# BaratiLab/LNS-Latent-Neural-PDE-Solver

Measured on AMD Instinct MI355X. Metric: rollout-steps/sec (encode+N latent steps+decode), NS2d 128^2 3-ch, higher is better.
Workload: dtype f32 (f16x2 split operands on the fp16 MFMA pipe, fp32 accumulate; fp32 tensors in HBM); 1 GPU; NS2d 128x128 3-channel, 64-step latent rollout, batch=64 per GPU (BASELINE.json configs[1]); preset=ns2d_128, batch_per_gpu=64, rollout_steps=64, global_batch=64, parallelism=trajectory-sharded x1, streams=propagator + 3 decode streams per GPU

## Files before the change

lns-latent-neural-pde-solver_amd/csrc/conv3_up2q.inc:

```
#define CONVUQ_SLAB 8192
#define CONVUQ_STEP 2
#define CONVUQ_EPS_BYTES 32768

size_t convuq_lds_bytes(const ConvArgs& a) {
    const size_t ns = a.Cin_pad / 8, pp1 = (size_t)a.PH * a.PW + 1;
    return ns * pp1 * 32 + CONVUQ_EPS_BYTES + ((size_t)a.Cin_pad * 2 + 64) * 4 + 16 + 64;
}
bool convuq_fits(const ConvArgs& a) {
    return a.ks == 3 && a.stride == 1 && a.dil == 1 && a.up2 && a.wb != nullptr && a.Cin_pad >= 16 && a.Cin_pad <= 64 &&
           (a.Cin_pad % 16) == 0 && (long)a.PH * a.PW <= 256 && !a.x_oct && a.b0 == 0 && a.res == nullptr &&
           (long)a.Cout * a.Hout * a.Wout * 4 < (1L << 31) && convuq_lds_bytes(a) <= 80 * 1024;
}

template <bool FUSE2>
__global__ __launch_bounds__(256, 2) void conv3_up2q_kernel(ConvArgs a) {
    constexpr int NTHR = 256, TM = 64, KC = 8, MT = 2, NT = 1, UB = 32, SLAB = CONVUQ_SLAB, NS_MAX = 8, STEP = CONVUQ_STEP;
    constexpr int NWQ = STEP * SLAB / 16 / NTHR;
    static_assert(2 * STEP * SLAB <= CONVUQ_EPS_BYTES && 18944 <= CONVUQ_EPS_BYTES, "the ring covers the epilogue scratch it aliases");
    extern __shared__ __attribute__((aligned(16))) char smem[];
    const int PH = a.PH, PW = a.PW, PLANE = PH * PW, PP1 = PLANE + 1;
    const int ns = a.Cin_pad / KC;
    const int xs_bytes = PP1 * UB;
    char* Xres = smem;
    char* ring = Xres + ns * xs_bytes;
    float* ssl = reinterpret_cast<float*>(ring + CONVUQ_EPS_BYTES);
    float* addv = ssl + a.Cin_pad * 2;
    unsigned* wmax = reinterpret_cast<unsigned*>(addv + 64);

    const int tid = threadIdx.x, lane = tid & 63, wn = tid >> 6;
    const int l31 = lane & 31, kh = lane >> 5;
    const int b = blockIdx.y;
    const int ct = blockIdx.x % a.cout_tiles, tile = blockIdx.x / a.cout_tiles;
    const int tx = tile % a.tiles_x, ty = tile / a.tiles_x;
    const int BW = 1 << a.bw_log2, BH = 128 >> a.bw_log2;
// ... 39 lines not shown
    };
    load_half(0);
    const int nstep = ns / STEP;
    u32x4 wq[NWQ];
    auto load_w = [&](int q) __attribute__((always_inline)) {
        const int qc = q < 4 * nstep ? q : 4 * nstep - 1;
        const int ph = qc / nstep, sp0 = (qc - ph * nstep) * STEP;
#pragma unroll
        for (int i = 0; i < NWQ; ++i) {
            const int idx = tid + i * NTHR, st = sp0 + (idx >> 9);
            wq[i] = __builtin_amdgcn_raw_buffer_load_b128(wr, (idx & 511) * 16, (st * 4 + ph) * SLAB, 0);
        }
    };
    auto write_w = [&](int slot) __attribute__((always_inline)) {
#pragma unroll
        for (int i = 0; i < NWQ; ++i) *reinterpret_cast<u32x4*>(ring + slot * (STEP * SLAB) + (tid + i * NTHR) * 16) = wq[i];
    };
    load_w(0);
    {
        float addreg = 0.0f;
        if (tid < TM) {
            const int co = ct * TM + tid, cc = co < a.Cout ? co : 0;
            addreg = (a.bias ? a.bias[cc] : 0.0f) + (a.badd ? a.badd[(long)b * a.Cout + cc] : 0.0f);
        }
        stage_ss_bound(a, b, ssl, wmax, tid, NTHR);
        if (tid < TM) addv[tid] = addreg;
    }
    __syncthreads();
    float xinv = 1.0f;
    uok *= f16x2_scale(block_bound(a, wmax), xinv);

    auto stage_half = [&](auto mode_tag, int h) __attribute__((always_inline)) {
        constexpr int MODE = decltype(mode_tag)::value;
#pragma unroll
        for (int sl = 0; sl < HS; ++sl) {
            const int s = h * HS + sl;
            if (s < ns) {
                unsigned hq[4], lq[4];
#pragma unroll
                for (int cp = 0; cp < 4; ++cp) {
                    float t[2];
#pragma unroll
                    for (int e = 0; e < 2; ++e) {
                        float v = pv[sl * KC + 2 * cp + e];
                        if (MODE >= 1) { const float2 st = *reinterpret_cast<const float2*>(ssl + 2 * (s * KC + 2 * cp + e)); v = v * st.x + st.y; }
                        if (MODE == 2) v = swish_fast(v);
// ... 2 lines not shown
                    split2_pair_f16(t[0], t[1], hq[cp], lq[cp]);
                }
                char* dst = Xres + s * xs_bytes + uslot;
                *reinterpret_cast<uint4*>(dst) = make_uint4(hq[0], hq[1], hq[2], hq[3]);
                *reinterpret_cast<uint4*>(dst + 16) = make_uint4(lq[0], lq[1], lq[2], lq[3]);
            }
        }
    };
    auto stage_all = [&](auto mode_tag) __attribute__((always_inline)) {
        stage_half(mode_tag, 0);
        if (ns > HS) { load_half(1); stage_half(mode_tag, 1); }
    };
    if (pro_mode == 2) stage_all(std::integral_constant<int, 2>{});
    else if (pro_mode == 1) stage_all(std::integral_constant<int, 1>{});
    else stage_all(std::integral_constant<int, 0>{});
    write_w(0);
    load_w(1);
    __syncthreads();

    const int p = wn * 32 + l31;
    const int boff = ((p >> a.bw_log2) * PW + (p & (BW - 1))) * UB;
    const int aoff0 = ((0 + kh) * TM + l31) * 16, aoff1 = ((2 + kh) * TM + l31) * 16;
    unsigned am = 0u;
#pragma unroll 1
    for (int ph = 0; ph < 4; ++ph) {
        const int pa = ph >> 1, pb = ph & 1;
        const int lt0 = ((0 + pa) * PW + kh + pb) * UB, lt1 = ((1 + pa) * PW + kh + pb) * UB;
        f32x16 acc_hi[MT][NT], acc_lo[MT][NT];
#pragma unroll
        for (int mt = 0; mt < MT; ++mt)
#pragma unroll
            for (int r = 0; r < 16; ++r) { acc_hi[mt][0][r] = 0.0f; acc_lo[mt][0][r] = 0.0f; }
#pragma unroll 1
        for (int t = 0; t < nstep; ++t) {
#pragma unroll
            for (int u = 0; u < STEP; ++u) {
                const char* Wslot = ring + (t & 1) * (STEP * SLAB) + u * SLAB;
                const char* Xs = Xres + (t * STEP + u) * xs_bytes + boff;
                uint4 af[2][2][MT], bf[2][2];
#pragma unroll
                for (int j = 0; j < 2; ++j)
#pragma unroll
                    for (int sp = 0; sp < 2; ++sp) {
#pragma unroll
                        for (int mt = 0; mt < MT; ++mt)
                            af[j][sp][mt] = *reinterpret_cast<const uint4*>(Wslot + (j ? aoff1 : aoff0) + sp * (4 * TM * 16) + mt * (32 * 16));
                        bf[j][sp] = *reinterpret_cast<const uint4*>(Xs + (j ? lt1 : lt0) + sp * 16);
                    }
#pragma unroll
                for (int j = 0; j < 2; ++j) {
#define LNS_UQ3(ACC, SA, SB)                                                                          \
    _Pragma("unroll") for (int mt = 0; mt < MT; ++mt)                                                 \
        ACC[mt][0] = __builtin_amdgcn_mfma_f32_32x32x16_f16(__builtin_bit_cast(f16x8, af[j][SA][mt]), \
                                                            __builtin_bit_cast(f16x8, bf[j][SB]), ACC[mt][0], 0, 0, 0);
                    LNS_UQ3(acc_hi, 0, 0)
                    LNS_UQ3(acc_lo, 0, 1)
                    LNS_UQ3(acc_lo, 1, 0)
#undef LNS_UQ3
                }
            }
            if (t + 1 < nstep) {
                write_w((t + 1) & 1);
                if (t + 2 < nstep) load_w(ph * nstep + t + 2);
            }
            __syncthreads();
        }
        int pix[NT];
        {
            const int oy = 2 * (ty * BH + (p >> a.bw_log2)) + pa, ox = 2 * (tx * BW + (p & (BW - 1))) + pb;
            pix[0] = (oy < a.Hout && ox < a.Wout) ? oy * a.Wout + ox : -1;
        }
        convb_epilogue<NT, FUSE2, MT, true, true, true, true>(a, acc_hi, acc_lo, pix, b, ct, kh, l31, tid, ring, xinv, am,
                                                        (a.bias || a.badd) ? addv : nullptr, (ty * a.tiles_x + tx) * 4 + ph, nullptr, 4);
        if (ph < 3) {
            load_w((ph + 1) * nstep);
            __syncthreads();
            write_w(0);
            load_w((ph + 1) * nstep + 1);
            __syncthreads();
        }
    }
    if (a.amax_out) amax_publish_block(a.amax_out, b, am, wmax);
}

hipError_t launch_conv_up2q(const ConvArgs& a, hipStream_t s) {
    if (!convuq_fits(a) || !has_act_bound(a)) return hipErrorInvalidValue;
    dim3 grid(a.tiles_x * a.tiles_y * a.cout_tiles, a.B);
    const size_t lds = convuq_lds_bytes(a);
    if (a.w2) hipLaunchKernelGGL((conv3_up2q_kernel<true>), grid, dim3(256), lds, s, a);
    else hipLaunchKernelGGL((conv3_up2q_kernel<false>), grid, dim3(256), lds, s, a);
    return hipGetLastError();
}
```

lns-latent-neural-pde-solver_amd/csrc/lns_engine.cpp:

```cpp
#include <algorithm>
#include <cmath>
#include <cstdarg>
#include <cstdio>
#include <cstdlib>
#include <cstring>
#include <memory>
#include <mutex>
#include <tuple>
#include <stdexcept>
#include <type_traits>

#include "lns_engine.h"
#include "lns_fold.h"

#define LNS_MAX_BATCH 65535

namespace lns {
void build_model(lns_engine* e);

static thread_local std::string g_create_error;

static std::string fmt(const char* f, ...) {
    char buf[1024];
    va_list ap;
// ... 45 lines not shown
    out.resize(len);
    for (int p = 0; p < len; ++p) {
        int u = p - pad_lo;
        int src = -1;
        if (p < virt + pad_lo + pad_hi) {
            if (u < 0 || u >= virt) {
                if (mode == LNS_PAD_CIRCULAR) { u %= virt; if (u < 0) u += virt; }
                else u = -1;
            }
            if (u >= 0) src = nearest_src(u, in, virt, scale);
        }
        out[p] = src;
    }
}

static void pack_conv_weight(float* dst, const float* src, int cout_off, int cout, int cin, int k, int Cin_pad,
                             int Cout_pad) {
    const int taps = k * k;
    for (int co = 0; co < cout; ++co)
        for (int ci = 0; ci < cin; ++ci)
            for (int t = 0; t < taps; ++t)
                dst[((size_t)t * Cin_pad + ci) * Cout_pad + cout_off + co] = src[((size_t)co * cin + ci) * taps + t];
}

struct ConvGeom { int variant, bw_log2, tiles_x, tiles_y, cout_tiles, PH, PW, Hout, Wout, kc_log2, sel_kc_log2; };

static bool conv_geometry(ConvGeom& g, int B, int Cout, int Hv, int Wv, int k, int stride, int dil, const int* pad,
                          int kc_log2_pack, int Cout_pad, int force_variant, bool need_wgm1 = false,
                          bool allow_bf16x3 = false, int Cin = 1 << 30, bool f16x2 = false, bool allow_thin = false,
                          int force_bw_log2 = -1 ) {
    g.Hout = (Hv + pad[0] + pad[1] - dil * (k - 1) - 1) / stride + 1;
    g.Wout = (Wv + pad[2] + pad[3] - dil * (k - 1) - 1) / stride + 1;
    if (g.Hout <= 0 || g.Wout <= 0) return false;
    std::vector<int> cands;
    if (force_variant >= 0) cands = {force_variant};
    else if (Cout <= 32) cands = {CV_S32};
    else if (Cout <= 64) cands = need_wgm1 ? std::vector<int>{CV_L64, CV_M64} : std::vector<int>{CV_L64, CV_M64, CV_S64};
    else if (getenv("LNS_CONV_USE_128")) cands = {CV_L128, CV_M128, CV_S64};
    else cands = {CV_L64, CV_M64, CV_S64};
    static const bool no_bf16x3 = getenv("LNS_CONV_FP32_MFMA") != nullptr;
    const bool use_b = allow_bf16x3 && !no_bf16x3 && k == 3 && stride == 1 && Cout > 32;
    if (force_variant < 0 && use_b) {
        cands.insert(cands.begin(), f16x2 ? (int)CV_F64 : (int)CV_B64);
    }
    static const bool no_b1 = getenv("LNS_CONV1_FP32_MFMA") != nullptr;
    if (force_variant < 0 && allow_bf16x3 && !no_bf16x3 && !no_b1 && k == 1 && stride == 1 && Cout > 32 && Cin >= 16)
// ... 237 lines not shown
        static const long min_hw = getenv("LNS_GN_FUSE_MIN_HW") ? atol(getenv("LNS_GN_FUSE_MIN_HW")) : (no_fold ? 1024 : 256);
        Op* prod = nullptr;
        for (size_t i = plan->ops.size(); i-- > 0;) {
            const int ty = plan->ops[i].type;
            if (ty == OP_TRACE || ty == OP_CONDBLK || ty == OP_CONDBASE || ty == OP_VECLIN) continue;
            prod = &plan->ops[i];
            break;
        }
        static const bool no_ragged = getenv("LNS_GN_NO_RAGGED") != nullptr;
        const bool ragged1 = !no_fold && !no_ragged && prod && prod->type == OP_CONV && !prod->conv.up2 &&
                             prod->conv.tiles_x * prod->conv.tiles_y == 1 && x.H * x.W < GN_TILE_PIXELS;
        static const bool no_ragged_tiles = getenv("LNS_GN_NO_RAGGED_TILES") != nullptr;
        const bool raggedN = !no_fold && !no_ragged && !no_ragged_tiles && prod && prod->type == OP_CONV && !prod->conv.up2 && !ragged1 &&
                             x.H * x.W > GN_TILE_PIXELS;
        const bool prod_ok = prod && prod->type == OP_CONV &&
                             (prod->variant == CV_F64 || prod->variant == CV_F32 || prod->variant == CV_B64 ||
                              (prod->variant == CV_B1 && !no_fold && prod->conv.ct_per_block == 0 && !prod->conv.w2 &&
                               ((x.H * x.W) % GN_TILE_PIXELS == 0 || ragged1 || raggedN)));
        if (stat_scratch && (!premul || ragged1 || raggedN) && prod_ok &&
            prod->conv.y == as_ptr<float>(x.ptr) && prod->conv.Cout == x.C && ((long)x.H * x.W >= min_hw || ragged1)) {
            const ConvArgs& c = prod->conv;
            const int BW = 1 << c.bw_log2, BH = GN_TILE_PIXELS / BW;
            const int um = c.up2 ? 2 : 1;
            const int tiles = c.tiles_x * c.tiles_y * (c.up2 ? 4 : 1);
            const bool exact = c.ks == 1 ? (c.tiles_x * GN_TILE_PIXELS == x.H * x.W && c.tiles_y == 1)
                                         : (c.tiles_x * BW * um == x.W && c.tiles_y * BH * um == x.H);
            if ((exact || ragged1 || raggedN) && (size_t)B * tiles * x.C * 8 <= stat_cap) {
                const int cg = x.C / groups;
                static const int fold_tiles = getenv("LNS_GN_FOLD_TILES") ? atoi(getenv("LNS_GN_FOLD_TILES")) : 2;
                const bool foldable = !no_fold && (exact || ragged1) && tiles <= fold_tiles && x.C <= 512 && (!premul || groups == 1) &&
                                      (groups == 1 || (cg <= 64 && (cg & (cg - 1)) == 0));
                const int li = (int)lazy_ops.size();
                lazy_done.push_back(0); lazy_folded.push_back(0);
                const uint64_t region = take_stat_region(name, li);
                prod->conv.stat_part = as_ptr<float>(region);
                op.gn_tile_part = as_ptr<const float>(region);
                op.gn_tiles = tiles;
                op.gn_count = ragged1 ? x.H * x.W : GN_TILE_PIXELS;
                if (ragged1) prod->conv.stat_count = x.H * x.W;
                if (!exact && !ragged1) {
                    op.gn_count = -1;
                    op.gn_geom = GnTileGeom{c.tiles_x, c.bw_log2, x.H, x.W, c.ks == 1 ? 1 : 0};
                    prod->conv.stat_count = -1;
                }
                if (prod->chunk_group > 0)
                    for (Op& o : plan->ops)
                        if (o.type == OP_CONV && o.chunk_group == prod->chunk_group) {
                            o.conv.stat_part = prod->conv.stat_part; o.conv.stat_count = prod->conv.stat_count;
                        }
                op.bytes = 2.0 * B * tiles * x.C * 8;
                lazy_ops.push_back(op);
                if (foldable) { x.gn_lazy = li; return; }
                lazy_done[li] = 1;
            }
        }
        plan->ops.push_back(op);
    }

    static bool can_fuse_1x1(const ConvPack& first, const ConvPack& second) {
        static const bool off = getenv("LNS_NO_FUSE_1X1") != nullptr;
        return !off && first.cout == 64 && second.k == 1 && second.cin == 64 && second.cout == 64;
// ... 1 lines not shown
    TRef emit_conv(const TRef& in, int pack_id, int k, int stride, int dil, const int* pad, int my, int mx,
                   int act_out, const TRef* res, uint64_t badd, const TRef* out_forced, const std::string& name,
                   int fuse_pack = -1, bool want_amax = true) {
        const ConvPack& pk = e->packs[pack_id];
        if (pk.cin != in.C) throw std::runtime_error(fmt("%s: input has %d channels, conv expects %d", name.c_str(), in.C, pk.cin));
        int Hv = in.vH ? in.vH : in.H, Wv = in.vW ? in.vW : in.W;
        static const bool fp32_only = getenv("LNS_CONV_FP32_MFMA") != nullptr;
        const bool up2 = k == 3 && stride == 1 && dil == 1 && in.vH == 2 * in.H && in.vW == 2 * in.W && pk.has_wu && pk.f16 &&
                         pad[0] == 1 && pad[1] == 1 && pad[2] == 1 && pad[3] == 1 && in.bounded() && pk.cout > 32 && !fp32_only;
        if (up2) { Hv = in.H; Wv = in.W; }
        ConvGeom g;
        const bool thin_ok = !res && !badd && act_out == ACT_NONE && fuse_pack < 0 && !in.vH &&
                             (in.act == ACT_NONE || (in.act == ACT_SWISH && in.ss != 0));
        if (!conv_geometry(g, B, pk.cout, Hv, Wv, k, stride, dil, pad, pk.kc_log2, pk.Cout_pad, -1, fuse_pack >= 0,
                           pk.has_wb && in.bounded(), pk.cin, pk.f16, thin_ok))
            throw std::runtime_error("no conv tiling for " + name);
        if (up2 && g.variant == CV_F32 &&
            !conv_geometry(g, B, pk.cout, Hv, Wv, k, stride, dil, pad, pk.kc_log2, pk.Cout_pad, CV_F64, fuse_pack >= 0,
                           pk.has_wb && in.bounded(), pk.cin, pk.f16, thin_ok))
            throw std::runtime_error("no conv tiling for " + name);
        if (up2 && g.variant != CV_F64) throw std::runtime_error("phase form needs the f16x2 64-cout tiles: " + name);
        bool quad = false;
        {
            static const bool no_quad = getenv("LNS_UP2_QUAD") == nullptr || getenv("LNS_UP2_RESIDENT") != nullptr;
            ConvGeom gq;
            if (up2 && !no_quad && !res && pk.Cin_pad <= 64 && pk.Cin_pad % 16 == 0 &&
                conv_geometry(gq, B, pk.cout, Hv, Wv, k, stride, dil, pad, pk.kc_log2, pk.Cout_pad, CV_F64, fuse_pack >= 0,
                              pk.has_wb && in.bounded(), pk.cin, pk.f16, thin_ok, 4)) {
                ConvArgs t;
                memset(&t, 0, sizeof t);
                t.ks = 3; t.stride = 1; t.dil = 1; t.up2 = 1; t.wb = &t; t.Cin_pad = pk.Cin_pad; t.PH = gq.PH; t.PW = gq.PW;
                t.Cout = pk.cout; t.Hout = 2 * in.H; t.Wout = 2 * in.W;
                if (convuq_fits(t)) { g = gq; quad = true; }
            }
        }
        if (in.act == ACT_GELU && ((g.variant != CV_F64 && g.variant != CV_F32) || up2 || fuse_pack >= 0))
            throw NoGeluPrologue("GELU prologue is only built into the f16x2 3x3 kernel: " + name);
        if (up2) { g.Hout = 2 * in.H; g.Wout = 2 * in.W; }
        const ConvVariantInfo vi = conv_variant_info(g.variant);
        const int BW = 1 << g.bw_log2, BH = vi.TN / BW;
        std::vector<int> rm, cm;
        if (k == 3) {
            build_axis_map(rm, (g.tiles_y - 1) * BH * stride + g.PH, in.H, Hv, up2 ? 0.0f : in.sch, pad[0], pad[1], my);
            build_axis_map(cm, (g.tiles_x - 1) * BW * stride + g.PW, in.W, Wv, up2 ? 0.0f : in.scw, pad[2], pad[3], mx);
        } else if (in.vH) throw std::runtime_error("1x1 conv of a resized tensor is not supported: " + name);
        TRef out;
        if (out_forced) out = *out_forced;
        else out = alloc_t(pk.cout, g.Hout, g.Wout);
        if (out.C != pk.cout || out.H != g.Hout || out.W != g.Wout)
            throw std::runtime_error(fmt("%s: output shape mismatch (%d,%d,%d) vs (%d,%d,%d)", name.c_str(), out.C, out.H,
                                         out.W, pk.cout, g.Hout, g.Wout));
// ... 50 lines not shown
        a.unscale = (cv_is_f16x2_3x3(g.variant) || g.variant == CV_B1) ? 1.0f / (up2 ? pk.wscale_up : pk.wscale) : 1.0f;
        if (in.ss != 0 && in.gn_bound > 0.0f) { a.amax_in_const = in.gn_bound; a.bound_final = 1; }
        else {
            a.amax_in = as_ptr<const unsigned>(in.amax); a.amax_in_const = in.amax_const;
            if (!in.amax && in.ss == 0) a.bound_final = 1;
        }
        out.amax = 0; out.amax_const = 0.0f; out.gn_bound = 0.0f;
        if ((want_amax && g.variant != CV_THIN) || out_forced) { out.amax = new_amax(name); a.amax_out = as_ptr<unsigned>(out.amax); }
        a.Cin_pad = pk.Cin_pad; a.Cout_pad = pk.Cout_pad; a.kc_log2 = g.sel_kc_log2;
        a.tiles_x = g.tiles_x; a.tiles_y = g.tiles_y; a.cout_tiles = g.cout_tiles; a.bw_log2 = g.bw_log2;
        a.PH = g.PH; a.PW = g.PW; a.B = B;
        a.ph_magic = g.PH > 1 ? (unsigned)((0x100000000ull + g.PH - 1) / g.PH) : 0u;
        if (up2) {
            static const bool res = getenv("LNS_UP2_RESIDENT") != nullptr;
            if (res) { a.up2 = 2; if (!convur_fits(a)) a.up2 = 1; }
            if (quad && convuq_fits(a)) a.up2 = 3;
        }
        op.flops = 2.0 * B * g.Hout * g.Wout * (double)pk.cout * pk.cin * k * k;
        op.bytes = 4.0 * B * ((double)in.C * in.H * in.W + (double)pk.cout * g.Hout * g.Wout * (res ? 2 : 1));
        {
            const double tiles = (double)B * g.tiles_x * g.tiles_y * g.cout_tiles * vi.TM * vi.TN;
            if (cv_is_f16x2_3x3(g.variant)) {
                op.mfma_flops = tiles * pk.Cin_pad * (up2 ? 4.0 * 4.0 : 10.0) * 3.0 * 2.0;
                op.form = up2 ? (fuse_pack >= 0 ? "f16x2 3x3 four-tap phase form + fused 1x1" : "f16x2 3x3 four-tap phase form")
                              : (fuse_pack >= 0 ? "f16x2 3x3 nine-tap + fused 1x1" : "f16x2 3x3 nine-tap");
                if (fuse_pack >= 0) op.mfma_flops += tiles * (up2 ? 4.0 : 1.0) * 64.0 * 3.0 * 2.0;
            } else if (g.variant == CV_B64 || g.variant == CV_B32) {
                op.mfma_flops = tiles * pk.Cin_pad * 10.0 * 6.0 * 2.0; op.form = "bf16x3 3x3 nine-tap";
            } else if (g.variant == CV_B1) {
                const int cp32 = (pk.Cin_pad + 31) / 32 * 32;
                op.mfma_flops = tiles * cp32 * (convb1_is_f16() ? 3.0 : 6.0) * 2.0;
                op.form = a.ct_per_block ? "f16x2 1x1 input-stationary" : (fuse_pack >= 0 ? "f16x2 1x1 + fused 1x1" : "f16x2 1x1 streaming");
                if (fuse_pack >= 0) op.mfma_flops += tiles * 64.0 * 3.0 * 2.0;
            } else if (g.variant == CV_THIN) {
                op.form = "thin 1x1 projection (VALU)";
            } else {
                op.mfma_flops = tiles * pk.Cin_pad * (double)(k * k) * 2.0 + (fuse_pack >= 0 ? tiles * 64.0 * 2.0 : 0.0);
                op.form = k == 3 ? "fp32 MFMA 3x3" : "fp32 MFMA 1x1";
            }
        }
        if (fuse_pack >= 0) {
            const ConvPack& p2 = e->packs[fuse_pack];
            if (!can_fuse_1x1(pk, p2)) throw std::runtime_error("cannot fuse 1x1 into " + name);
            a.w2 = as_ptr<const float>(wt(p2.w_off));
            a.bias2 = p2.has_bias ? as_ptr<const float>(wt(p2.b_off)) : nullptr;
            a.Cout2_pad = p2.Cout_pad;
            {
// ... 1304 lines not shown
        if (n == "fa_fused" && (value < 0 || value > 3)) return LNS_EINVAL;
        const bool changed = n == "fa_fused" ? e->opt_fa_fused != (int)value : e->opt_fa_fused_gpb != (int)value;
        if (changed) {
            DeviceGuard dg(e);
            for (auto* m : {&e->enc_plans, &e->dec_plans}) {
                for (auto& kv : *m) if (kv.second.d_consts) (void)hipFree(kv.second.d_consts);
                m->clear();
            }
        }
        if (n == "fa_fused") e->opt_fa_fused = (int)value;
        else e->opt_fa_fused_gpb = (int)value;
    }
    else if (n == "fold_linear") {
        if (value != 0 && value != 1) { e->err = "fold_linear: 0 (the pair as it stands) or 1 (one conv on the composed weights)"; return LNS_EINVAL; }
        if (e->opt_fold_linear != (int)value) {
            DeviceGuard dg(e);
            for (auto* m : {&e->enc_plans, &e->dec_plans}) {
                for (auto& kv : *m) if (kv.second.d_consts) (void)hipFree(kv.second.d_consts);
                m->clear();
            }
        }
        e->opt_fold_linear = (int)value;
    }
    else if (n == "fa_chunk_mb") {
        if (value < 0 || value > 4096) return LNS_EINVAL;
        if (e->opt_fa_chunk_mb != (int)value) {
            DeviceGuard dg(e);
            for (auto* m : {&e->enc_plans, &e->dec_plans}) {
                for (auto& kv : *m) if (kv.second.d_consts) (void)hipFree(kv.second.d_consts);
                m->clear();
            }
        }
        e->opt_fa_chunk_mb = (int)value;
    }
    else if (n == "prop_priority") {
        if (e->opt_prop_priority != (value != 0)) { DeviceGuard dg(e); release_overlap_objects(e); }
        e->opt_prop_priority = value != 0;
    } else { e->err = "unknown option: " + n; return LNS_EINVAL; }
    e->ran.clear(); e->ran_ws = nullptr; e->ran_B = 0;
    return LNS_OK;
}

int lns_latent_shape(const lns_engine* e, int* C, int* H, int* W) {
    if (!e || e->enc.empty()) return LNS_EINVAL;
    if (C) *C = e->lat_C;
    if (H) *H = e->lat_H;
// ... 485 lines not shown
    if (name && cap > 0) { strncpy(name, t.name.c_str(), cap - 1); name[cap - 1] = 0; }
    if (ms) *ms = t.ms;
    if (launches) *launches = t.launches;
    if (flops) *flops = t.flops;
    if (bytes) *bytes = t.bytes;
    return LNS_OK;
}

int lns_timing_mfma_flops(const lns_engine* e, int i, double* mfma_flops) {
    if (e && i == -1 && mfma_flops) { *mfma_flops = e->timing_overhead_ms * 1e3; return LNS_OK; }
    if (!e || i < 0 || i >= (int)e->timing.size() || !mfma_flops) return LNS_EINVAL;
    *mfma_flops = e->timing[i].mfma_flops;
    return LNS_OK;
}

int lns_build_has(const char* feature) {
    if (!feature) return -1;
    if (!strcmp(feature, "experimental")) return build_has_experimental() ? 1 : 0;
    if (!strcmp(feature, "train_wgrad_split")) return 1;
    if (!strcmp(feature, "train_clip")) return 1;
    if (!strcmp(feature, "train_ops")) return 1;
    if (!strcmp(feature, "rollout_select")) return 1;
    if (!strcmp(feature, "rollout_ensemble")) return 1;
#ifdef LNS_DIAG
    if (!strcmp(feature, "diag")) return 1;
#else
    if (!strcmp(feature, "diag")) return 0;
#endif
    return -1;
}
static thread_local std::string g_op_error;
#define OPCHK(call)                                                                                   \
    do { hipError_t err__ = (call);                                                                   \
         if (err__ != hipSuccess) { g_op_error = fmt("%s: %s", #call, hipGetErrorString(err__)); fprintf(stderr, "lns_op: %s\n", g_op_error.c_str()); return LNS_EHIP; } } while (0)

struct OpConv {
    ConvArgs a;
    int variant = -1;
    float* dw = nullptr;
    int* dmaps = nullptr;
    unsigned* damax = nullptr;
    void release() { (void)hipFree(dw); (void)hipFree(dmaps); (void)hipFree(damax); dw = nullptr; dmaps = nullptr; damax = nullptr; }
};

static int op_conv_prepare(OpConv& oc, const float* x, int B, int Cin, int Hin, int Win, int Hv, int Wv,
                           const float* w_host, const float* bias_host, int Cout, int ksize, int stride, int dilation,
                           int pad_t, int pad_b, int pad_l, int pad_r, int mode_y, int mode_x, const float* ss, int act_in,
                           int act_out, const float* residual, const float* badd, float* y, int tile_variant, hipStream_t stream) {
    if (!x || !w_host || !y || (ksize != 1 && ksize != 3)) return LNS_EINVAL;
    if (act_in != ACT_NONE && act_in != ACT_SWISH) return LNS_EINVAL;
    OPCHK(init_kernels());
    const int layout = tile_variant >= 0 ? (tile_variant & 0x300) : 0;
    if (tile_variant >= 0) tile_variant &= 0xff;
    const bool stationary = tile_variant == 8;
    if (stationary) tile_variant = CV_B1;
    const bool w8 = tile_variant == 19;
    const bool forced = tile_variant >= 0;
    if (w8) tile_variant = CV_F64;
    const bool up2r = tile_variant == 18;
    const bool up2q = tile_variant == 20;
    const bool up2 = tile_variant == 17 || up2r || up2q;
    if (up2) {
        if (ksize != 3 || stride != 1 || dilation != 1 || Hv != 2 * Hin || Wv != 2 * Win || pad_t != 1 || pad_b != 1 || pad_l != 1 || pad_r != 1) return LNS_EINVAL;
        tile_variant = CV_F64; Hv = Hin; Wv = Win;
    }
    ConvPack pk;
    pk.cin = Cin; pk.cout = Cout; pk.k = ksize;
    pk.kc_log2 = ksize == 3 ? 3 : 5;
    pk.Cin_pad = (Cin + (1 << pk.kc_log2) - 1) / (1 << pk.kc_log2) * (1 << pk.kc_log2);
    pk.Cout_pad = Cout <= 32 ? 32 : (Cout <= 64 ? 64 : (Cout + 127) / 128 * 128);
    if (tile_variant >= 0) {
        const int TM = conv_variant_info(tile_variant).TM;
        pk.Cout_pad = (Cout + TM - 1) / TM * TM;
        if (pk.Cout_pad < 32) pk.Cout_pad = 32;
    }
    if (Hv <= 0) Hv = Hin;
    if (Wv <= 0) Wv = Win;
    const int pad[4] = {pad_t, pad_b, pad_l, pad_r};
    ConvGeom g;
    if (!conv_geometry(g, B, Cout, Hv, Wv, ksize, stride, dilation, pad, pk.kc_log2, pk.Cout_pad, tile_variant, false, false, 1 << 30, false,
                       false, up2q ? 4 : -1)) return LNS_EINVAL;
    const ConvVariantInfo vi = conv_variant_info(g.variant);
    const int BW = 1 << g.bw_log2, BH = vi.TN / BW;
// ... 41 lines not shown
        a.map_pad[0] = pad_t; a.map_pad[1] = pad_l;
        a.map_ext[0] = Hin + pad_t + pad_b; a.map_ext[1] = Win + pad_l + pad_r;
    }
    a.vec4 = (ksize == 1 && ((Hin * Win) % 4 == 0)) ? 1 : 0;
    a.y = y; a.y_bs = (long)Cout * g.Hout * g.Wout; a.Cout = Cout; a.Hout = g.Hout; a.Wout = g.Wout;
    a.res = residual; a.res_bs = a.y_bs; a.badd = badd;
    a.ks = ksize; a.stride = stride; a.dil = dilation; a.Cin_pad = pk.Cin_pad; a.Cout_pad = pk.Cout_pad;
    a.unscale = (cv_is_f16x2_3x3(g.variant) || g.variant == CV_B1) ? 1.0f / wscale : 1.0f;
    a.up2 = up2 ? 1 : 0;
    OPCHK(hipMalloc(reinterpret_cast<void**>(&oc.damax), (size_t)B * LNS_AMAX_SUB * 4));
    OPCHK(hipMemsetAsync(oc.damax, 0, (size_t)B * LNS_AMAX_SUB * 4, stream));
    OPCHK(launch_amax(x, a.x_bs, (long)Cin * Hin * Win, B, oc.damax, stream));
    a.amax_in = oc.damax;
    a.kc_log2 = g.sel_kc_log2; a.tiles_x = g.tiles_x; a.tiles_y = g.tiles_y; a.cout_tiles = g.cout_tiles;
    a.bw_log2 = g.bw_log2; a.PH = g.PH; a.PW = g.PW; a.B = B;
    a.ph_magic = g.PH > 1 ? (unsigned)((0x100000000ull + g.PH - 1) / g.PH) : 0u;
    if (up2r) {
        a.up2 = 2;
        if (!convur_fits(a)) return LNS_EINVAL;
    }
    if (up2q) {
        a.up2 = 3;
        if (!convuq_fits(a)) return LNS_EINVAL;
    }
    a.w8 = w8 ? 1 : (forced ? -1 : 0);
    a.x_oct = (layout & 0x100) ? 1 : 0; a.y_oct = (layout & 0x200) ? 1 : 0;
    if ((a.x_oct && (Cin & 7)) || (a.y_oct && (Cout & 7))) return LNS_EINVAL;
    if (stationary) {
        if (pk.Cin_pad > 64) return LNS_EINVAL;
        a.ct_per_block = g.cout_tiles < 3 ? g.cout_tiles : 3;
    }
    oc.variant = g.variant;
    return LNS_OK;
}

int lns_op_conv2d(const float* x, int B, int Cin, int Hin, int Win, int Hv, int Wv, const float* w_host,
                  const float* bias_host, int Cout, int ksize, int stride, int dilation, int pad_t, int pad_b, int pad_l,
                  int pad_r, int mode_y, int mode_x, const float* ss, int act_in, int act_out, const float* residual,
                  const float* badd, float* y, int tile_variant, void* stream, unsigned* amax_out) {
    OpConv oc;
    const int rc = op_conv_prepare(oc, x, B, Cin, Hin, Win, Hv, Wv, w_host, bias_host, Cout, ksize, stride, dilation, pad_t,
                                   pad_b, pad_l, pad_r, mode_y, mode_x, ss, act_in, act_out, residual, badd, y, tile_variant,
                                   static_cast<hipStream_t>(stream));
    if (rc) { oc.release(); return rc; }
    oc.a.amax_out = amax_out;
    hipStream_t s = static_cast<hipStream_t>(stream);
// ... 363 lines not shown
```

lns-latent-neural-pde-solver_amd/csrc/lns_engine.h:

```cpp
#pragma once
#include <map>
#include <string>
#include <vector>

#include "../../include/lns.h"
#include "lns_kernels.h"

namespace lns {

struct Param {
    std::string key;
    std::vector<int64_t> shape;
    std::vector<float> host;
    bool is_buffer = false;
    bool is_set = false;
    size_t numel() const { size_t n = 1; for (auto s : shape) n *= (size_t)s; return n; }
};

struct ConvPack {
    std::vector<std::string> wkeys;
    std::vector<std::string> bkeys;
    std::vector<int> couts;
    int cin = 0, cout = 0, k = 1;
    bool has_bias = false;
// ... 97 lines not shown
    std::vector<lns::Param> params;
    std::map<std::string, int> pindex;
    std::vector<lns::ConvPack> packs;
    std::vector<lns::VecPack> vecs;
    std::vector<lns::Layer> enc, dec, prop;
    int lat_C = 0, lat_H = 0, lat_W = 0;
    float* d_weights = nullptr;
    size_t weights_floats = 0;
    bool finalized = false;
    int device = -1;
    std::map<long, lns::Plan> enc_plans, dec_plans, prop_plans;
    void* side_stream = nullptr;
    std::vector<hipStream_t> dec_streams;
    std::vector<hipEvent_t> events;
    int opt_decode_group = 1;
    int opt_decode_streams = 3;
    int opt_eval_max_steps = 1024;
    int opt_overlap = 1;
    int opt_prop_priority = 0;
    int opt_fa_chunk_mb = 0;
    int opt_fa_fused = 2;
    int opt_fa_fused_gpb = 0;
    int opt_fold_linear = 1;
    struct RanRec { int kind; long key; size_t arena_off; };
    std::vector<RanRec> ran;
    const void* ran_ws = nullptr;
    int ran_B = 0;
    int opt_track_nonfinite = 0;
    int opt_train_wgrad = 0;
    unsigned* d_sticky = nullptr;
    bool sticky_armed = false;
    bool trace_on = false;
    std::vector<lns::TraceRec> trace;
    bool timing_on = false;
    std::vector<lns::TimeRec> timing;
    double timing_overhead_ms = -1.0;
};
```

lns-latent-neural-pde-solver_amd/csrc/lns_kernels.hip:

```cpp
#include <cstdlib>
#include <type_traits>

#include "lns_kernels.h"

namespace lns {

#ifndef LNS_CONV_STORE_AUX
#define LNS_CONV_STORE_AUX 0
#endif
#ifndef LNS_NTS_CONV3F
#define LNS_NTS_CONV3F 0
#endif
#ifndef LNS_NTS_CONV1F
#define LNS_NTS_CONV1F 0
#endif
#ifndef LNS_SAND_STORE_AUX
#define LNS_SAND_STORE_AUX 0
#endif
typedef float f32x16 __attribute__((ext_vector_type(16)));

__device__ __forceinline__ float gelu_erfc(float v) {
    const float z = fabsf(v) * 0.70710678118654752440f;
    const float t = __builtin_amdgcn_rcpf(fmaf(0.5f, z, 1.0f));
    float p = 0.17087277f;
// ... 722 lines not shown
    if (a.dbg_ts && threadIdx.x == 0) {                                                               \
        long long* d_ = a.dbg_ts + ((long)blockIdx.y * gridDim.x + blockIdx.x) * 8;                   \
        for (int i_ = 0; i_ < 6; ++i_) d_[i_] = ts_[i_];                                              \
        d_[6] = __builtin_amdgcn_s_getreg((31 << 11) | 4);                                            \
        d_[7] = __builtin_amdgcn_s_getreg((31 << 11) | 20);                                           \
    }
#else
#define LNS_TS_DECL
#define LNS_TSTAMP(i)
#define LNS_TS_DUMP
#endif
#if defined(LNS_TS) && LNS_TS == 2
#define LNS_ETS(i) if (ets) { __builtin_amdgcn_sched_barrier(0); ets[i] = wall_clock64(); __builtin_amdgcn_sched_barrier(0); }
#define LNS_ETS_ARG , ts_
#else
#define LNS_ETS(i)
#define LNS_ETS_ARG , nullptr
#endif

template <int NT, bool FUSE2, int MT = 2, bool STATS = true, bool OCT = true, bool SHALF = false, bool NORES = false, bool NTS = false>
__device__ __forceinline__ void convb_epilogue(const ConvArgs& a, f32x16 (&acc_hi)[MT][NT], f32x16 (&acc_lo)[MT][NT],
                                               const int (&pix)[NT], int b, int ct, int kh, int l31, int tid, char* lds,
                                               float xinv, unsigned& am, const float* addv = nullptr, int sp_tile = -1, long long* ets = nullptr,
                                               int tile_mult = 1) {
    constexpr int TM = 32 * MT, NTHR = 256;
    static_assert(!FUSE2 || MT == 2, "the fused second 1x1 needs all 64 channels of a pixel in one wave");
    LNS_ETS(0)
    float w2v[FUSE2 ? TM * TM / NTHR : 1];
    if (FUSE2) {
#pragma unroll
        for (int u = 0; u < TM * TM / NTHR; ++u) {
            const int i = tid + u * NTHR, k = i / TM, co2 = i - k * TM;
            w2v[u] = a.w2[(long)k * a.Cout2_pad + co2];
        }
    }
    f32x16 acc[MT][NT];
#pragma unroll
    for (int mt = 0; mt < MT; ++mt)
#pragma unroll
        for (int nt = 0; nt < NT; ++nt)
#pragma unroll
            for (int r = 0; r < 16; ++r)
                acc[mt][nt][r] = ((acc_hi[mt][nt][r] + acc_lo[mt][nt][r]) * a.unscale) * xinv;
    const int HWo = a.Hout * a.Wout;
    float* yb = y_base(a, b);
    const float* rb = (!NORES && a.res) ? a.res + (long)b * a.res_bs : nullptr;
    float rv[MT][NT][16];
// ... 260 lines not shown
#pragma unroll
    for (int nt = 0; nt < NT; ++nt) {
        if (pix[nt] < 0) continue;
#pragma unroll
        for (int mt = 0; mt < MT; ++mt) {
            const int cob = ct * TM + mt * 32 + 4 * kh;
            float* yp = yb + ((long)cob * HWo + pix[nt]);
#pragma unroll
            for (int r = 0; r < 16; ++r) {
                const int co = cob + (r & 3) + 8 * (r >> 2);
                if (co < a.Cout) {
                    const int ro = ((r & 3) + 8 * (r >> 2)) * HWo;
                    float v = acc[mt][nt][r];
                    if (rb) v += rv[mt][nt][r];
                    yp[ro] = v;
                    am = max(am, abs_bits(v));
                    if (SHALF) acc[mt][nt][r] = v;
                    else if (stats) sb[(mt * 32 + drow(r, kh)) * SROW + (tid >> 6) * 33 + l31] = v;
                }
            }
        }
    }
    LNS_ETS(4)
    constexpr int SROWS = SHALF ? 32 : TM;
    if (stats)
    for (int hf = 0; hf < (SHALF ? MT : 1); ++hf) {
        if (SHALF) {
            if (hf) __syncthreads();
#pragma unroll
            for (int mt = 0; mt < MT; ++mt)
                if (mt == hf) {
#pragma unroll
                    for (int r = 0; r < 16; ++r) sb[drow(r, kh) * SROW + (tid >> 6) * 33 + l31] = acc[mt][0][r];
                }
        }
        unsigned* smask = reinterpret_cast<unsigned*>(sb + SROWS * SROW);
        const unsigned long long have = __builtin_amdgcn_ballot_w64(pix[0] >= 0);
        if (a.stat_count && (tid & 63) == 0) smask[tid >> 6] = (unsigned)have;
        __syncthreads();
        const int c = tid >> 2, q = tid & 3;
        if (c < SROWS) {
        const float* row = sb + c * SROW + q * 33;
        float v[32];
#pragma unroll
        for (int i = 0; i < 32; ++i) v[i] = row[i];
        float mean, m2;
// ... 1181 lines not shown
        if (two) LNS_LAUNCH_F16X2(2, false, 1, 9, grid);
        else LNS_LAUNCH_F16X2(1, false, 1, 9, grid);
        return hipGetLastError();
    }
#undef LNS_LAUNCH_F16X2
    if (variant == CV_B32) {
        if (a.w2) return hipErrorInvalidValue;
        const size_t lds = convb_lds_bytes(a, 32, 3, 2);
        if (two) hipLaunchKernelGGL((conv3_bf16x3_kernel<1, 2, false, 1>), grid, dim3(256), lds, s, a);
        else hipLaunchKernelGGL((conv3_bf16x3_kernel<1, 1, false, 1>), grid, dim3(256), lds, s, a);
        return hipGetLastError();
    }
    const size_t lds = convb_lds_bytes(a, 64, 3, 2);
    if (a.w2) {
        if (two) hipLaunchKernelGGL((conv3_bf16x3_kernel<1, 2, true>), grid, dim3(256), lds, s, a);
        else hipLaunchKernelGGL((conv3_bf16x3_kernel<1, 1, true>), grid, dim3(256), lds, s, a);
    } else {
        if (two) hipLaunchKernelGGL((conv3_bf16x3_kernel<1, 2, false>), grid, dim3(256), lds, s, a);
        else hipLaunchKernelGGL((conv3_bf16x3_kernel<1, 1, false>), grid, dim3(256), lds, s, a);
    }
    return hipGetLastError();
}

#ifdef LNS_EXPERIMENTAL
#include "conv3_pc.inc"
#include "conv3_up2r.inc"
#include "conv3_up2q.inc"
#include "conv3_w8.inc"
bool build_has_experimental() { return true; }
#else
bool build_has_experimental() { return false; }
size_t convuq_lds_bytes(const ConvArgs&) { return 0; }
bool convuq_fits(const ConvArgs&) { return false; }
hipError_t launch_conv_up2q(const ConvArgs&, hipStream_t) { return hipErrorInvalidValue; }
size_t convpc_lds_bytes(const ConvArgs&, int) { return 0; }
bool convpc_geom_fits(const ConvArgs&, int) { return false; }
bool convpc_fits(const ConvArgs&, int) { return false; }
hipError_t launch_conv_pc(int, const ConvArgs&, hipStream_t) { return hipErrorInvalidValue; }
bool convur_fits(const ConvArgs&) { return false; }
size_t convur_lds_bytes(const ConvArgs&) { return 0; }
hipError_t launch_conv_up2r(const ConvArgs&, hipStream_t) { return hipErrorInvalidValue; }
bool convw8_fits(const ConvArgs&) { return false; }
hipError_t launch_conv_w8(const ConvArgs&, hipStream_t) { return hipErrorInvalidValue; }
#endif

__global__ __launch_bounds__(256) void conv1_thin_kernel(ConvArgs a) {
    __shared__ float wsm[4 * 512];
    __shared__ float2 ssm[512];
    const int tid = threadIdx.x, b = blockIdx.y + a.b0;
    const int HW = a.Hin * a.Win, C = a.Cin, CO = a.Cout;
    const bool has_ss = a.ss != nullptr;
    for (int i = tid; i < CO * C; i += 256) {
        const int co = i / C, c = i - co * C;
        wsm[co * 512 + c] = a.w[(long)c * a.Cout_pad + co];
    }
    for (int i = tid; i < C; i += 256)
        ssm[i] = has_ss ? make_float2(a.ss[((long)b * C + i) * 2], a.ss[((long)b * C + i) * 2 + 1]) : make_float2(1.0f, 0.0f);
// ... 2272 lines not shown

__global__ __launch_bounds__(256) void amax_sticky_kernel(const unsigned* amax, int n, unsigned* flag) {
    bool bad = false;
    for (int i = threadIdx.x; i < n; i += 256) bad = bad || ((amax[i] >> 23) & 0xffu) == 0xffu;
    if (__builtin_amdgcn_ballot_w64(bad) != 0ull && (threadIdx.x & 63) == 0) atomicOr(flag, 1u);
}
hipError_t launch_amax_sticky(const unsigned* amax, int n, unsigned* flag, hipStream_t s) {
    hipLaunchKernelGGL(amax_sticky_kernel, dim3(1), dim3(256), 0, s, amax, n, flag);
    return hipGetLastError();
}

__global__ void empty_kernel() {}
hipError_t launch_empty(hipStream_t s) {
    hipLaunchKernelGGL(empty_kernel, dim3(1), dim3(64), 0, s);
    return hipGetLastError();
}

hipError_t init_kernels() {
    hipError_t e;
    const int maxlds = 160 * 1024;
#define LNS_SET_LDS(k)                                                                            \
    e = hipFuncSetAttribute(reinterpret_cast<const void*>(k), hipFuncAttributeMaxDynamicSharedMemorySize, maxlds); \
    if (e != hipSuccess) return e;
#ifdef LNS_EXPERIMENTAL
    LNS_SET_LDS((conv3_up2q_kernel<true>))
    LNS_SET_LDS((conv3_up2q_kernel<false>))
    LNS_SET_LDS(conv3_w8_kernel<1>)
    LNS_SET_LDS(conv3_w8_kernel<2>)
    LNS_SET_LDS((conv3_up2r_kernel<true>))
    LNS_SET_LDS((conv3_up2r_kernel<false>))
    LNS_SET_LDS((conv3_pc_kernel<1, 1>))
    LNS_SET_LDS((conv3_pc_kernel<1, 2>))
    LNS_SET_LDS((conv3_pc_kernel<2, 1>))
    LNS_SET_LDS((conv3_pc_kernel<2, 2>))
#endif
    LNS_SET_LDS((conv_mfma_kernel<2, 4, 2, 2, 3, false, 4>))
    LNS_SET_LDS((conv_mfma_kernel<2, 4, 2, 2, 3, false, 8>))
    LNS_SET_LDS((conv_mfma_kernel<2, 4, 2, 2, 1, true, 16>))
    LNS_SET_LDS((conv_mfma_kernel<2, 4, 2, 2, 1, false, 16>))
    LNS_SET_LDS((conv_mfma_kernel<2, 2, 1, 4, 3, false, 4>))
    LNS_SET_LDS((conv_mfma_kernel<2, 2, 1, 4, 3, false, 4, true>))
    LNS_SET_LDS((conv_mfma_kernel<2, 2, 1, 4, 3, false, 8, true>))
    LNS_SET_LDS((conv_mfma_kernel<2, 2, 1, 4, 1, true, 16, true>))
    LNS_SET_LDS((conv_mfma_kernel<2, 2, 1, 4, 1, false, 16, true>))
    LNS_SET_LDS((conv_mfma_kernel<2, 2, 1, 4, 3, false, 8>))
    LNS_SET_LDS((conv_mfma_kernel<2, 2, 1, 4, 1, true, 16>))
    LNS_SET_LDS((conv_mfma_kernel<2, 2, 1, 4, 1, false, 16>))
    LNS_SET_LDS((conv_mfma_kernel<2, 2, 2, 2, 3, false, 4>))
    LNS_SET_LDS((conv_mfma_kernel<2, 2, 2, 2, 3, false, 8>))
// ... 98 lines not shown
```

Baseline: 39650 trajectory-steps/s.

## Enable quad-phase upsample conv by default with fused per-tile GroupNorm stats

Moves the quad-phase up2 3x3 conv kernel out of the experimental build and makes it the default for non-fused layers with enough tiles. The non-fused path now streams the weight ring continuously across all four phases instead of re-priming it between phases. It also computes GroupNorm partial mean/M2 per channel in-register across the four phases, using permlane/DPP reductions, and merges them into one stat entry per tile. The aim is to drop extra stat passes and ring refill stalls, at the cost of more register pressure and new numeric merge logic. An env/option knob allows disabling it.

Result: no change. 39650 trajectory-steps/s (-0.0%).

```diff
diff --git a/lns-latent-neural-pde-solver_amd/csrc/conv3_up2q.inc b/lns-latent-neural-pde-solver_amd/csrc/conv3_up2q.inc
--- a/lns-latent-neural-pde-solver_amd/csrc/conv3_up2q.inc
+++ b/lns-latent-neural-pde-solver_amd/csrc/conv3_up2q.inc
@@ -8,8 +8,38 @@
 }
 bool convuq_fits(const ConvArgs& a) {
     return a.ks == 3 && a.stride == 1 && a.dil == 1 && a.up2 && a.wb != nullptr && a.Cin_pad >= 16 && a.Cin_pad <= 64 &&
-           (a.Cin_pad % 16) == 0 && (long)a.PH * a.PW <= 256 && !a.x_oct && a.b0 == 0 && a.res == nullptr &&
+           (a.Cin_pad % 16) == 0 && (long)a.PH * a.PW <= 256 && !a.x_oct && !a.y_oct && a.b0 == 0 && a.res == nullptr &&
            (long)a.Cout * a.Hout * a.Wout * 4 < (1L << 31) && convuq_lds_bytes(a) <= 80 * 1024;
+}
+
+__device__ __forceinline__ void convuq_wave_stats(const f32x16 (&x)[2][1], int l31, int kh, int& ch, float& mean, float& m2) {
+    float mu[16], q[16];
+#pragma unroll
+    for (int r = 0; r < 16; ++r) {
+        const auto sw = __builtin_amdgcn_permlane16_swap(__float_as_uint(x[0][0][r]), __float_as_uint(x[1][0][r]), false, false);
+        const float u = __uint_as_float(sw[0]), v = __uint_as_float(sw[1]), d = u - v;
+        mu[r] = 0.5f * (u + v);
+        q[r] = 0.5f * (d * d);
+    }
+#define LNS_UQ_HALVE(H, CTRL, HALFN)                                                              \
+    {                                                                                             \
+        const bool up = (l31 & H) != 0;                                                           \
+        _Pragma("unroll") for (int i = 0; i < H; ++i) {                                           \
+            const float gm = up ? mu[i] : mu[i + H], gq = up ? q[i] : q[i + H];                   \
+            const float km = up ? mu[i + H] : mu[i], kq = up ? q[i + H] : q[i];                   \
+            const float rm = dpp_quad<CTRL>(gm), rq = dpp_quad<CTRL>(gq), d = km - rm;            \
+            mu[i] = 0.5f * (km + rm);                                                             \
+            q[i] = (kq + rq) + (d * d) * HALFN;                                                   \
+        }                                                                                         \
+    }
+    LNS_UQ_HALVE(8, 0x140, 1.0f)
+    LNS_UQ_HALVE(4, 0x141, 2.0f)
+    LNS_UQ_HALVE(2, 0x4E, 4.0f)
+    LNS_UQ_HALVE(1, 0xB1, 8.0f)
+#undef LNS_UQ_HALVE
+    ch = (l31 >> 4) * 32 + drow(l31 & 15, kh);
+    mean = mu[0];
+    m2 = q[0];
 }
 
 template <bool FUSE2>
@@ -95,6 +125,7 @@
         if (tid < TM) {
             const int co = ct * TM + tid, cc = co < a.Cout ? co : 0;
             addreg = (a.bias ? a.bias[cc] : 0.0f) + (a.badd ? a.badd[(long)b * a.Cout + cc] : 0.0f);
+            if (!FUSE2 && !a.bias && !a.badd) addreg = -0.0f;
         }
         stage_ss_bound(a, b, ssl, wmax, tid, NTHR);
         if (tid < TM) addv[tid] = addreg;
@@ -143,6 +174,8 @@
     const int boff = ((p >> a.bw_log2) * PW + (p & (BW - 1))) * UB;
     const int aoff0 = ((0 + kh) * TM + l31) * 16, aoff1 = ((2 + kh) * TM + l31) * 16;
     unsigned am = 0u;
+    float st_m[4] = {0.0f, 0.0f, 0.0f, 0.0f}, st_q[4] = {0.0f, 0.0f, 0.0f, 0.0f};
+    int st_ch = 0;
 #pragma unroll 1
     for (int ph = 0; ph < 4; ++ph) {
         const int pa = ph >> 1, pb = ph & 1;
@@ -154,9 +187,10 @@
             for (int r = 0; r < 16; ++r) { acc_hi[mt][0][r] = 0.0f; acc_lo[mt][0][r] = 0.0f; }
 #pragma unroll 1
         for (int t = 0; t < nstep; ++t) {
+            const int q = ph * nstep + t, cur = (FUSE2 ? t : q) & 1;
 #pragma unroll
             for (int u = 0; u < STEP; ++u) {
-                const char* Wslot = ring + (t & 1) * (STEP * SLAB) + u * SLAB;
+                const char* Wslot = ring + cur * (STEP * SLAB) + u * SLAB;
                 const char* Xs = Xres + (t * STEP + u) * xs_bytes + boff;
                 uint4 af[2][2][MT], bf[2][2];
 #pragma unroll
@@ -180,9 +214,9 @@
 #undef LNS_UQ3
                 }
             }
-            if (t + 1 < nstep) {
-                write_w((t + 1) & 1);
-                if (t + 2 < nstep) load_w(ph * nstep + t + 2);
+            if (FUSE2 ? t + 1 < nstep : q + 1 < 4 * nstep) {
+                write_w(cur ^ 1);
+                if (FUSE2 ? t + 2 < nstep : q + 2 < 4 * nstep) load_w(q + 2);
             }
             __syncthreads();
         }
@@ -191,14 +225,51 @@
             const int oy = 2 * (ty * BH + (p >> a.bw_log2)) + pa, ox = 2 * (tx * BW + (p & (BW - 1))) + pb;
             pix[0] = (oy < a.Hout && ox < a.Wout) ? oy * a.Wout + ox : -1;
         }
-        convb_epilogue<NT, FUSE2, MT, true, true, true, true>(a, acc_hi, acc_lo, pix, b, ct, kh, l31, tid, ring, xinv, am,
-                                                        (a.bias || a.badd) ? addv : nullptr, (ty * a.tiles_x + tx) * 4 + ph, nullptr, 4);
-        if (ph < 3) {
-            load_w((ph + 1) * nstep);
+        if constexpr (FUSE2) {
+            convb_epilogue<NT, true, MT, true, true, true, true>(a, acc_hi, acc_lo, pix, b, ct, kh, l31, tid, ring, xinv, am,
+                                                                 (a.bias || a.badd) ? addv : nullptr, (ty * a.tiles_x + tx) * 4 + ph, nullptr, 4);
+            if (ph < 3) {
+                load_w((ph + 1) * nstep);
+                __syncthreads();
+                write_w(0);
+                load_w((ph + 1) * nstep + 1);
+                __syncthreads();
+            }
+        } else {
+            int ctv = ct;
+            asm volatile("" : "+s"(ctv));
+            __builtin_assume(addv != nullptr);
+            __builtin_assume((long)a.Cout * (a.Hout * a.Wout) * 4 < (1L << 31));
+            convb_epilogue<NT, false, MT, false, false, true, true>(a, acc_hi, acc_lo, pix, b, ctv, kh, l31, tid, ring, xinv, am,
+                                                                    addv, -1, nullptr, 1, true);
+            if (a.stat_part) {
+                float pm, pq;
+                convuq_wave_stats(acc_hi, l31, kh, st_ch, pm, pq);
+                if (ph == 0) { st_m[0] = pm; st_q[0] = pq; }
+                else if (ph == 1) { st_m[1] = pm; st_q[1] = pq; }
+                else if (ph == 2) { st_m[2] = pm; st_q[2] = pq; }
+                else { st_m[3] = pm; st_q[3] = pq; }
+            }
+        }
+    }
+    if constexpr (!FUSE2) {
+        if (a.stat_part) {
+            float2* tab = reinterpret_cast<float2*>(ring);
+#pragma unroll
+            for (int k = 0; k < 4; ++k) tab[(k * 4 + wn) * TM + st_ch] = make_float2(st_m[k], st_q[k]);
             __syncthreads();
-            write_w(0);
-            load_w((ph + 1) * nstep + 1);
-            __syncthreads();
+            const int co = ct * TM + tid;
+            if (tid < TM && co < a.Cout) {
+                float2 acc = tab[tid];
+#pragma unroll
+                for (int k = 1; k < 16; ++k) {
+                    const float2 o = tab[k * TM + tid];
+                    const float d = o.x - acc.x;
+                    acc.x += d * (1.0f / (float)(k + 1));
+                    acc.y = (acc.y + o.y) + (d * d) * (32.0f * (float)k / (float)(k + 1));
+                }
+                *reinterpret_cast<float2*>(a.stat_part + (((long)b * (a.tiles_x * a.tiles_y) + (ty * a.tiles_x + tx)) * a.Cout + co) * 2) = acc;
+            }
         }
     }
     if (a.amax_out) amax_publish_block(a.amax_out, b, am, wmax);
@@ -208,7 +279,12 @@
     if (!convuq_fits(a) || !has_act_bound(a)) return hipErrorInvalidValue;
     dim3 grid(a.tiles_x * a.tiles_y * a.cout_tiles, a.B);
     const size_t lds = convuq_lds_bytes(a);
+#ifdef LNS_EXPERIMENTAL
     if (a.w2) hipLaunchKernelGGL((conv3_up2q_kernel<true>), grid, dim3(256), lds, s, a);
-    else hipLaunchKernelGGL((conv3_up2q_kernel<false>), grid, dim3(256), lds, s, a);
+    else
+#else
+    if (a.w2) return hipErrorInvalidValue;
+#endif
+    hipLaunchKernelGGL((conv3_up2q_kernel<false>), grid, dim3(256), lds, s, a);
     return hipGetLastError();
 }
diff --git a/lns-latent-neural-pde-solver_amd/csrc/lns_engine.cpp b/lns-latent-neural-pde-solver_amd/csrc/lns_engine.cpp
--- a/lns-latent-neural-pde-solver_amd/csrc/lns_engine.cpp
+++ b/lns-latent-neural-pde-solver_amd/csrc/lns_engine.cpp
@@ -91,6 +91,8 @@
             for (int t = 0; t < taps; ++t)
                 dst[((size_t)t * Cin_pad + ci) * Cout_pad + cout_off + co] = src[((size_t)co * cin + ci) * taps + t];
 }
+
+static const int UP2_QUAD_MIN_TILES = 32;
 
 struct ConvGeom { int variant, bw_log2, tiles_x, tiles_y, cout_tiles, PH, PW, Hout, Wout, kc_log2, sel_kc_log2; };
 
@@ -374,7 +376,8 @@
             const ConvArgs& c = prod->conv;
             const int BW = 1 << c.bw_log2, BH = GN_TILE_PIXELS / BW;
             const int um = c.up2 ? 2 : 1;
-            const int tiles = c.tiles_x * c.tiles_y * (c.up2 ? 4 : 1);
+            const bool quad1 = c.up2 == 3 && !c.w2;
+            const int tiles = c.tiles_x * c.tiles_y * (c.up2 && !quad1 ? 4 : 1);
             const bool exact = c.ks == 1 ? (c.tiles_x * GN_TILE_PIXELS == x.H * x.W && c.tiles_y == 1)
                                          : (c.tiles_x * BW * um == x.W && c.tiles_y * BH * um == x.H);
             if ((exact || ragged1 || raggedN) && (size_t)B * tiles * x.C * 8 <= stat_cap) {
@@ -388,7 +391,7 @@
                 prod->conv.stat_part = as_ptr<float>(region);
                 op.gn_tile_part = as_ptr<const float>(region);
                 op.gn_tiles = tiles;
-                op.gn_count = ragged1 ? x.H * x.W : GN_TILE_PIXELS;
+                op.gn_count = ragged1 ? x.H * x.W : quad1 ? 4 * GN_TILE_PIXELS : GN_TILE_PIXELS;
                 if (ragged1) prod->conv.stat_count = x.H * x.W;
                 if (!exact && !ragged1) {
                     op.gn_count = -1;
@@ -436,11 +439,15 @@
         if (up2 && g.variant != CV_F64) throw std::runtime_error("phase form needs the f16x2 64-cout tiles: " + name);
         bool quad = false;
         {
-            static const bool no_quad = getenv("LNS_UP2_QUAD") == nullptr || getenv("LNS_UP2_RESIDENT") != nullptr;
+            static const bool env_off = getenv("LNS_NO_UP2_QUAD") != nullptr;
+            static const bool env_all = build_has_experimental() && getenv("LNS_UP2_QUAD") != nullptr;
+            static const bool resident = getenv("LNS_UP2_RESIDENT") != nullptr;
+            const int mode = e->opt_up2_quad >= 0 ? e->opt_up2_quad : (env_off ? 0 : 1);
             ConvGeom gq;
-            if (up2 && !no_quad && !res && pk.Cin_pad <= 64 && pk.Cin_pad % 16 == 0 &&
+            if (up2 && (mode > 0 || env_all) && !resident && !res && (fuse_pack < 0 || env_all) && pk.Cin_pad <= 64 && pk.Cin_pad % 16 == 0 &&
                 conv_geometry(gq, B, pk.cout, Hv, Wv, k, stride, dil, pad, pk.kc_log2, pk.Cout_pad, CV_F64, fuse_pack >= 0,
-                              pk.has_wb && in.bounded(), pk.cin, pk.f16, thin_ok, 4)) {
+                              pk.has_wb && in.bounded(), pk.cin, pk.f16, thin_ok, 4) &&
+                (mode == 2 || env_all || gq.tiles_x * gq.tiles_y >= UP2_QUAD_MIN_TILES)) {
                 ConvArgs t;
                 memset(&t, 0, sizeof t);
                 t.ks = 3; t.stride = 1; t.dil = 1; t.up2 = 1; t.wb = &t; t.Cin_pad = pk.Cin_pad; t.PH = gq.PH; t.PW = gq.PW;
@@ -537,7 +544,8 @@
             const double tiles = (double)B * g.tiles_x * g.tiles_y * g.cout_tiles * vi.TM * vi.TN;
             if (cv_is_f16x2_3x3(g.variant)) {
                 op.mfma_flops = tiles * pk.Cin_pad * (up2 ? 4.0 * 4.0 : 10.0) * 3.0 * 2.0;
-                op.form = up2 ? (fuse_pack >= 0 ? "f16x2 3x3 four-tap phase form + fused 1x1" : "f16x2 3x3 four-tap phase form")
+                op.form = up2 ? (fuse_pack >= 0 ? "f16x2 3x3 four-tap phase form + fused 1x1"
+                                                : a.up2 == 3 ? "f16x2 3x3 four-tap quad-phase form" : "f16x2 3x3 four-tap phase form")
                               : (fuse_pack >= 0 ? "f16x2 3x3 nine-tap + fused 1x1" : "f16x2 3x3 nine-tap");
                 if (fuse_pack >= 0) op.mfma_flops += tiles * (up2 ? 4.0 : 1.0) * 64.0 * 3.0 * 2.0;
             } else if (g.variant == CV_B64 || g.variant == CV_B32) {
@@ -1888,6 +1896,17 @@
         }
         e->opt_fold_linear = (int)value;
     }
+    else if (n == "up2_quad") {
+        if (value < 0 || value > 2) { e->err = "up2_quad: 0 (never), 1 (the per-layer rule) or 2 (wherever the quad-phase form fits)"; return LNS_EINVAL; }
+        if (e->opt_up2_quad != (int)value) {
+            DeviceGuard dg(e);
+            for (auto* m : {&e->enc_plans, &e->dec_plans}) {
+                for (auto& kv : *m) if (kv.second.d_consts) (void)hipFree(kv.second.d_consts);
+                m->clear();
+            }
+        }
+        e->opt_up2_quad = (int)value;
+    }
     else if (n == "fa_chunk_mb") {
         if (value < 0 || value > 4096) return LNS_EINVAL;
         if (e->opt_fa_chunk_mb != (int)value) {
@@ -2419,6 +2438,7 @@
     if (!strcmp(feature, "train_ops")) return 1;
     if (!strcmp(feature, "rollout_select")) return 1;
     if (!strcmp(feature, "rollout_ensemble")) return 1;
+    if (!strcmp(feature, "up2_quad")) return 1;
 #ifdef LNS_DIAG
     if (!strcmp(feature, "diag")) return 1;
 #else
@@ -2455,7 +2475,8 @@
     const bool forced = tile_variant >= 0;
     if (w8) tile_variant = CV_F64;
     const bool up2r = tile_variant == 18;
-    const bool up2q = tile_variant == 20;
+    const bool up2q_fused = tile_variant == 21;
+    const bool up2q = tile_variant == 20 || up2q_fused;
     const bool up2 = tile_variant == 17 || up2r || up2q;
     if (up2) {
         if (ksize != 3 || stride != 1 || dilation != 1 || Hv != 2 * Hin || Wv != 2 * Win || pad_t != 1 || pad_b != 1 || pad_l != 1 || pad_r != 1) return LNS_EINVAL;
@@ -2543,6 +2564,10 @@
     if (up2q) {
         a.up2 = 3;
         if (!convuq_fits(a)) return LNS_EINVAL;
+        if (up2q_fused) {
+            if (build_has_experimental()) return LNS_EINVAL;
+            a.w2 = oc.dw; a.Cout2_pad = 64; a.w2scale = 1.0f;
+        }
     }
     a.w8 = w8 ? 1 : (forced ? -1 : 0);
     a.x_oct = (layout & 0x100) ? 1 : 0; a.y_oct = (layout & 0x200) ? 1 : 0;
diff --git a/lns-latent-neural-pde-solver_amd/csrc/lns_engine.h b/lns-latent-neural-pde-solver_amd/csrc/lns_engine.h
--- a/lns-latent-neural-pde-solver_amd/csrc/lns_engine.h
+++ b/lns-latent-neural-pde-solver_amd/csrc/lns_engine.h
@@ -143,6 +143,7 @@
     int opt_fa_fused = 2;
     int opt_fa_fused_gpb = 0;
     int opt_fold_linear = 1;
+    int opt_up2_quad = -1;
     struct RanRec { int kind; long key; size_t arena_off; };
     std::vector<RanRec> ran;
     const void* ran_ws = nullptr;
diff --git a/lns-latent-neural-pde-solver_amd/csrc/lns_kernels.hip b/lns-latent-neural-pde-solver_amd/csrc/lns_kernels.hip
--- a/lns-latent-neural-pde-solver_amd/csrc/lns_kernels.hip
+++ b/lns-latent-neural-pde-solver_amd/csrc/lns_kernels.hip
@@ -768,7 +768,7 @@
 __device__ __forceinline__ void convb_epilogue(const ConvArgs& a, f32x16 (&acc_hi)[MT][NT], f32x16 (&acc_lo)[MT][NT],
                                                const int (&pix)[NT], int b, int ct, int kh, int l31, int tid, char* lds,
                                                float xinv, unsigned& am, const float* addv = nullptr, int sp_tile = -1, long long* ets = nullptr,
-                                               int tile_mult = 1) {
+                                               int tile_mult = 1, bool hand_back = false) {
     constexpr int TM = 32 * MT, NTHR = 256;
     static_assert(!FUSE2 || MT == 2, "the fused second 1x1 needs all 64 channels of a pixel in one wave");
     LNS_ETS(0)
@@ -1075,6 +1075,12 @@
         }
     }
     LNS_ETS(4)
+    if (SHALF && hand_back) {
+#pragma unroll
+        for (int mt = 0; mt < MT; ++mt)
+#pragma unroll
+            for (int nt = 0; nt < NT; ++nt) acc_hi[mt][nt] = acc[mt][nt];
+    }
     constexpr int SROWS = SHALF ? 32 : TM;
     if (stats)
     for (int hf = 0; hf < (SHALF ? MT : 1); ++hf) {
@@ -2302,17 +2308,14 @@
     return hipGetLastError();
 }
 
+#include "conv3_up2q.inc"
 #ifdef LNS_EXPERIMENTAL
 #include "conv3_pc.inc"
 #include "conv3_up2r.inc"
-#include "conv3_up2q.inc"
 #include "conv3_w8.inc"
 bool build_has_experimental() { return true; }
 #else
 bool build_has_experimental() { return false; }
-size_t convuq_lds_bytes(const ConvArgs&) { return 0; }
-bool convuq_fits(const ConvArgs&) { return false; }
-hipError_t launch_conv_up2q(const ConvArgs&, hipStream_t) { return hipErrorInvalidValue; }
 size_t convpc_lds_bytes(const ConvArgs&, int) { return 0; }
 bool convpc_geom_fits(const ConvArgs&, int) { return false; }
 bool convpc_fits(const ConvArgs&, int) { return false; }
@@ -4631,9 +4634,9 @@
 #define LNS_SET_LDS(k)                                                                            \
     e = hipFuncSetAttribute(reinterpret_cast<const void*>(k), hipFuncAttributeMaxDynamicSharedMemorySize, maxlds); \
     if (e != hipSuccess) return e;
+    LNS_SET_LDS((conv3_up2q_kernel<false>))
 #ifdef LNS_EXPERIMENTAL
     LNS_SET_LDS((conv3_up2q_kernel<true>))
-    LNS_SET_LDS((conv3_up2q_kernel<false>))
     LNS_SET_LDS(conv3_w8_kernel<1>)
     LNS_SET_LDS(conv3_w8_kernel<2>)
     LNS_SET_LDS((conv3_up2r_kernel<true>))
```
